# stablecabal/gyre

Hardware: AMD Instinct MI355X
Metric: SD1.5 512px 50-step images/sec (node) (higher is better)
Workload: dtype bf16

## Files before the change

gyre_amd/_lib.py:

```python
from __future__ import annotations

import ctypes as C
import os
from typing import Optional

import torch

_HERE = os.path.dirname(os.path.abspath(__file__))
MAX_LEVELS = 8

F32, BF16, F16 = 0, 1, 2
_TORCH_DTYPE = {torch.float32: F32, torch.bfloat16: BF16, torch.float16: F16}
LIB_PATHS = {BF16: os.environ.get("GYRE_HIP_LIB") or os.path.join(_HERE, "libgyre_hip.so"),
             F16: os.environ.get("GYRE_HIP_LIB_F16") or os.path.join(_HERE, "libgyre_hip_f16.so")}
LIB_PATH = LIB_PATHS[BF16]
_default_storage = F16 if os.environ.get("GYRE_STORAGE", "").lower() in ("f16", "fp16", "float16", "half") else BF16
STORAGE_TORCH_DTYPE = {BF16: torch.bfloat16, F16: torch.float16}


def default_storage() -> int:
    return _default_storage


def set_default_storage(storage: int) -> int:
# ... 139 lines not shown
    "gyre_op_repack_conv_weight": (_i, [_vp, _vp, _i, _i, _i, _i, _i, _vp]),
    "gyre_op_repack_conv_weight_scaled": (_i, [_vp, _vp, _i, _i, _i, _i, _i, _i, _f, _vp]),
    "gyre_op_repack_linear_weight": (_i, [_vp, _vp, _i, _i, _i, _vp]),
    "gyre_op_repack_bias": (_i, [_vp, _vp, _i, _i, _vp]),
    "gyre_op_repack_lora": (_i, [_vp, _vp, _i, _i, _i, _i, _i, _i, _i, _f, _i, C.POINTER(LoraPair), _vp]),
    "gyre_op_attention": (_i, [_vp, _vp, _i, _vp, _i, _vp, _i, _i, _i, _i, _i, _i, _vp, _i]),
    "gyre_op_qkv": (_i, [_vp, _vp, _i, _i, _vp, _i, _vp, _vp, _i]),
    "gyre_op_attention_ex": (_i, [_vp, _vp, _i, _vp, _i, _vp, _i, _i, _i, _i, _i, _i, _vp, _i, _i]),
    "gyre_op_groupnorm_bwd_workspace": (_sz, [_i, _i, _i, _i]),
    "gyre_op_groupnorm_bwd": (_i, [_vp, _vp, _vp, _i, _i, _i, _i, _i, _vp, _vp, _f, _i, _vp, _vp, _vp, _sz, _vp, _vp]),
    "gyre_op_layernorm_bwd": (_i, [_vp, _vp, _vp, _i, _i, _vp, _f, _vp, _vp]),
    "gyre_op_geglu_bwd": (_i, [_vp, _vp, _vp, _i, _i, _vp]),
    "gyre_op_attention_bwd_workspace": (_sz, [_i, _i, _i, _i, _i]),
    "gyre_op_attention_bwd": (_i, [_vp, _vp, _i, _vp, _i, _vp, _i, _vp, _i, _vp, _i, _i, _i, _i, _i, _i, _i, _vp, _sz,
                                   _vp, _i, _vp, _i, _vp, _i]),
    "gyre_op_tome_workspace": (_sz, [_i, _i, _i]),
    "gyre_op_tome_merge": (_i, [_vp, _vp, _i, _vp, _i, _i, _i, _i, _i, _vp, _sz, _vp, _vp, _i, _vp, _vp]),
    "gyre_op_tome_merge_ex": (_i, [_vp, _vp, _i, _vp, _i, _i, _i, _i, _i, _vp, _sz, _vp, _vp, _i, _vp, _vp, _vp, _vp]),
    "gyre_op_tome_unmerge": (_i, [_vp, _vp, _i, _i, _i, _i, _vp, _vp, _vp, _vp, _i]),
    "gyre_op_timestep_embedding": (_i, [_vp, _vp, _i, _i, _i, _f, _vp]),
    "gyre_op_rowvec_linear": (_i, [_vp, _vp, _i, _i, _vp, _vp, _i, _i, _vp, _i]),
    "gyre_op_timestep_linear": (_i, [_vp, _vp, _i, _i, _i, _f, _vp, _vp, _vp, _i, _vp, _i]),
    "gyre_op_cross_attention_block": (_i, [_vp, _vp, _i, _i, _i, _i, _vp, _vp, _f, _vp, _vp, _vp, _i, _i, _vp, _vp, _vp, _sz, _vp, _vp]),
    "gyre_op_nchw_to_nhwc": (_i, [_vp, _vp, _i, _i, _i, _i, _i, _vp]),
    "gyre_op_copy_probe": (_i, [_vp, _vp, _vp, _sz]),
    "gyre_op_pixel_unshuffle8": (_i, [_vp, _vp, _i, _i, _i, _i, _i, _vp]),
    "gyre_op_avgpool2": (_i, [_vp, _vp, _i, _i, _i, _i, _vp]),
    "gyre_op_relu": (_i, [_vp, _vp, _sz]),
}
EXPORTED_SYMBOLS = tuple(_SIGS)

_libs: dict = {}
import threading as _threading
_tls = _threading.local()


def lib(storage: Optional[int] = None) -> C.CDLL:
    storage = _default_storage if storage is None else storage
    l = _libs.get(storage)
    if l is None:
        path = LIB_PATHS[storage]
        if not os.path.exists(path):
            raise GyreError(f"{path} is missing: run `python -c 'import __graft_entry__ as g; g.build()'` "
                            f"(hipcc --offload-arch=gfx950).  There is no non-HIP fallback.")
        try:
            l = C.CDLL(path, mode=getattr(os, "RTLD_LOCAL", 0) | getattr(os, "RTLD_NOW", 2))
# ... 69 lines not shown
```

gyre_amd/build.py:

```python
from __future__ import annotations

import os
import subprocess
import sys
from concurrent.futures import ThreadPoolExecutor

HERE = os.path.dirname(os.path.abspath(__file__))
CSRC = os.path.join(HERE, "csrc")
LIB = os.path.join(HERE, "libgyre_hip.so")
LIB_F16 = os.path.join(HERE, "libgyre_hip_f16.so")
SOURCES = ["kernels_elem.hip", "kernels_gemm.hip", "kernels_gemm4s.hip", "kernels_gemm_ar.hip", "kernels_gemm_sm.hip", "kernels_conv_out.hip", "kernels_attn.hip", "kernels_xattn.hip", "kernels_tome.hip", "kernels_bwd.hip", "kernels_t2i.hip", "kernels_lora.hip", "model.hip", "model_vjp.hip", "model_t2i.hip"]
HEADERS = ["common.h", "kernels.h", "gemm_shared.h", "model_impl.h", os.path.join("..", "..", "include", "gyre_hip.h")]
FLAGS = ["--offload-arch=gfx950", "-O3", "-std=c++17", "-fPIC", "-mcode-object-version=5",
         "-Wno-unused-result", "-fno-gpu-rdc",
         "-mllvm", "-pragma-unroll-threshold=1000000"]


PER_FILE_FLAGS = {"kernels_attn.hip": ["-mllvm", "-amdgpu-mfma-vgpr-form=1"]}

RESOURCE_FILES = ("kernels_attn.hip", "kernels_gemm.hip", "kernels_gemm4s.hip", "kernels_gemm_ar.hip", "kernels_gemm_sm.hip")
SCRATCH_ALLOWED = ("k_attn3ILi80E", "k_gemm4s")
RESOURCES_JSON = os.path.join(HERE, "build", "kernel_resources.json")


def _hipcc() -> str:
    for c in (os.environ.get("HIPCC"), "/opt/rocm/bin/hipcc", "hipcc"):
        if c and (os.path.isabs(c) and os.path.exists(c) or not os.path.isabs(c)):
            return c
    raise RuntimeError("hipcc not found")


def _stale(out: str, deps) -> bool:
    if not os.path.exists(out):
        return True
    t = os.path.getmtime(out)
    return any(os.path.getmtime(d) > t for d in deps)


def _record_resources(source: str, remarks: str) -> None:
    import json
    import re
    import threading
    kernels, cur = {}, None
# ... 87 lines not shown
```

gyre_amd/csrc/kernels.h:

```cpp
#pragma once
#include "common.h"

int launch_nchw_to_nhwc(hipStream_t st, const void* x, int dtype, int B, int C, int HW, int Cpad, bf16_t* y);
int launch_add_nchw_into_nhwc(hipStream_t st, const void* r, int dtype, int B, int C, int HW, int Cpad, bf16_t* y);
int launch_ctx_to_bf16(hipStream_t st, const void* x, int dtype, size_t n, bf16_t* y);
int launch_dup_batch(hipStream_t st, const void* src, void* dst, size_t outer, size_t inner_bytes);
int launch_add_f32(hipStream_t st, float* y, const float* x, size_t n);
int launch_verify_hints(hipStream_t st, const int64_t* t, int B, int check_t, const void* x, size_t bytes_per_half, int check_pairs, int* flag);
int launch_timestep_embedding(hipStream_t st, const int64_t* t, int B, int dim, int flip, float shift, float* out);
int launch_rowvec_linear(hipStream_t st, float* x, int B, int K, const bf16_t* W, const float* bias, int N,
                         int act_in_silu, float* out, int ldo);
int launch_timestep_linear(hipStream_t st, const int64_t* t, int B, int dim, int flip, float shift, float* emb_scratch,
                           const bf16_t* W, const float* bias, int N, float* out, int ldo);

struct GnParams {
    const bf16_t* x; const bf16_t* x2; int C1;
    int B, HW, C, G;
    const float* gamma; const float* beta; float eps; int silu;
    float* partial;
    float* scale_shift;
    int nchunks;
    bf16_t* y;
    float* mean_rstd = nullptr;
    const float* cs_x = nullptr; int cs_x_chunks = 0;
// ... 7 lines not shown
long gemm_planner_state();
enum : int {
    GEMM_DBG_NO_SM            = 0x20,
    GEMM_DBG_SM_NO_SPLITK     = 0x40,
    GEMM_DBG_NO_SC_FOLD       = 0x80,
    GEMM_DBG_CONV_ZERO_PAGE   = 0x200,
    GEMM_DBG_NO_4S            = 0x400,
    GEMM_DBG_NO_LN_FOLD       = 0x800,
    GEMM_DBG_NO_GN_FOLD       = 0x1000,
    GEMM_DBG_NO_XATTN         = 0x2000,
    GEMM_DBG_NO_GEGLU_4S      = 0x4000,
    GEMM_DBG_LN_STATS_PASS    = 0x8000,
    GEMM_DBG_GEGLU_NO_LN_FOLD = 0x10000,
    GEMM_DBG_GN_STATS_PASS    = 0x20000,
    GEMM_DBG_NO_128x160       = 0x40000,
    GEMM_DBG_NO_CS_128x160    = 0x100000,
    GEMM_DBG_NO_AR            = 0x200000,
    GEMM_DBG_AR_ALL           = 0x400000,
    GEMM_DBG_NO_4S_128_TILES  = 0x800000,
    GEMM_DBG_TWO_STAGE_LINEAR = 0x1000000,
    GEMM_DBG_DEEP_RING        = 0x2000000,
    GEMM_DBG_NO_W_BLOCK       = 0x4000000,
    GEMM_DBG_TWO_STAGE_CONV   = 0x8000000,
};
int launch_groupnorm_stats(hipStream_t st, const GnParams& p);
int launch_groupnorm_apply(hipStream_t st, const GnParams& p);
bool gn_use_small(int HW, int C, int C1, int G);
bool gn_accepts_colstats(const GnParams& p);
int launch_groupnorm_small(hipStream_t st, const GnParams& p);
int launch_gn_fold(hipStream_t st, const GnParams& p, const bf16_t* W, const float* bias, int N, bf16_t* Wf, float* bf);
int launch_layernorm(hipStream_t st, const bf16_t* x, int M, int C, const float* gamma, const float* beta, float eps,
                     bf16_t* y);
int launch_layernorm_stats(hipStream_t st, const bf16_t* x, int M, int C, float eps, float* stats);

int launch_nhwc_to_nchw_f32(hipStream_t st, const bf16_t* x, int B, int C, int HW, int Cpad, float* y);
int launch_repack_conv(hipStream_t st, const void* w, int dtype, int O, int I, int KH, int KW, int Ipad, bf16_t* out,
                       float scale = 1.f);
int launch_repack_linear(hipStream_t st, const void* w, int dtype, int O, int I, int geglu_interleave, bf16_t* out);
int launch_cast_f32(hipStream_t st, const void* w, int dtype, size_t n, int geglu_interleave, float* out, float scale = 1.f);
int launch_copy_probe(hipStream_t st, const void* src, void* dst, size_t bytes);
#define GYRE_LORA_MAX_PAIRS 8
struct LoraArgs {
    const void* up[GYRE_LORA_MAX_PAIRS];
    const void* down[GYRE_LORA_MAX_PAIRS];
    int dtype[GYRE_LORA_MAX_PAIRS];
    int rank[GYRE_LORA_MAX_PAIRS];
// ... 102 lines not shown
    bool always_check = false;
    int ablation = 0;
    double flops = 0, bytes = 0;
};
AttnPlan attn_plan(const AttnParams& p, int variant);
constexpr int ATTN_PLAN_INTS = 12, ATTN_BWD_PLAN_INTS = 10;
int launch_attention(hipStream_t st, const AttnParams& p);

struct XattnParams {
    const bf16_t* x; int ldx;
    const bf16_t* wq;
    const float* q_colsum; const float* q_bias;
    const float* ln_parts; int ln_nparts; const float* ln_stats; float ln_eps;
    const bf16_t* k; const bf16_t* vt; int ldvt;
    const bf16_t* wo; const float* bo;
    bf16_t* out; int ldo;
    float* rowstat_out;
    int M, rows_per_sample, Nk, heads;
};

bool xattn_supports(int C, int heads, int Nq, int Nk, int M);
int launch_xattn(hipStream_t st, const XattnParams& p, int C);

struct GnBwdParams {
    const bf16_t* x; const bf16_t* x2; int C1;
    int B, HW, C, G;
    const float* gamma; const float* beta; float eps; int silu;
    const bf16_t* dy;
    const bf16_t* addend;
    bf16_t* dx; bf16_t* dx2;
    float* partial = nullptr; const float* fwd_partial = nullptr; int nchunks = 0;
};
size_t gn_bwd_workspace_bytes(int B, int HW, int C, int G);
int launch_groupnorm_bwd(hipStream_t st, GnBwdParams p, void* ws);
int launch_layernorm_bwd(hipStream_t st, const bf16_t* x, const bf16_t* dy, int M, int C, const float* gamma, float eps,
                         const bf16_t* addend, bf16_t* dx);
int launch_geglu_bwd(hipStream_t st, const bf16_t* pre, const bf16_t* dy, size_t M, int F, bf16_t* dpre);
int launch_pool2_sum(hipStream_t st, const bf16_t* du, int B, int H, int W, int Hu, int Wu, int C, bf16_t* dx);
int launch_zero_stuff2(hipStream_t st, const bf16_t* dy, int B, int Ho, int Wo, int H, int W, int C, bf16_t* dz);
int launch_add_bf16(hipStream_t st, bf16_t* y, const bf16_t* x, size_t n);
int launch_conv_weight_t(hipStream_t st, const bf16_t* w, int O, int I, bf16_t* wt);
int launch_transpose(hipStream_t st, const bf16_t* in, int ld_in, int R, int C, bf16_t* out, int ld_out, int batch,
                     size_t bs_in, size_t bs_out);
struct AttnBwdParams {
    const bf16_t* q; int ldq;
    const bf16_t* k; int ldk;
// ... 35 lines not shown
```

gyre_amd/csrc/model.hip:

```cpp
#include "model_impl.h"

static thread_local std::string g_err;
static thread_local int64_t g_launches = 0;
void gyre_set_error(const std::string& msg) { g_err = msg; }
int64_t& gyre_launch_counter() { return g_launches; }
extern "C" const char* gyre_last_error(void) { return g_err.c_str(); }
extern "C" int gyre_abi_version(void) { return GYRE_ABI_VERSION; }
extern "C" int gyre_storage_dtype(void) { return GYRE_STORAGE_DTYPE; }
extern "C" int64_t gyre_last_launch_count(void) { return g_launches; }

namespace {
struct ProfRec { hipEvent_t a, b; int kclass; double flops, bytes; };
struct ProfState {
    unsigned long long mask = 0;
    std::vector<ProfRec> recs;
    std::vector<std::pair<hipEvent_t, hipEvent_t>> pool;
};
thread_local ProfState g_prof;
static_assert(KC_COUNT <= 64, "profiler mask is 64 bits wide");
}
GyreProfScope::GyreProfScope(int kclass, hipStream_t st, double flops, double bytes) : st_(st) {
    if (!(g_prof.mask >> kclass & 1ull)) return;
    hipEvent_t a, b;
    if (!g_prof.pool.empty()) { a = g_prof.pool.back().first; b = g_prof.pool.back().second; g_prof.pool.pop_back(); }
// ... 752 lines not shown
                      int n_parts, void* ws, size_t ws_bytes, void* y) {
    if (!x || !w || !y || !gamma || !beta || !ws) GYRE_FAIL(GYRE_ERR_INVALID, "null argument");
    GemmParams p;
    if (qkv_tokens > 0 && (!vt_out || M % qkv_tokens || N != 3 * K || geglu)) GYRE_FAIL(GYRE_ERR_INVALID, "bad fused Q|K|V arguments");
    ln_linear_problem(p, M, K, N, geglu, qkv_tokens, ldt);
    p.A = (const bf16_t*)x; p.W = (const bf16_t*)w; p.bias = bias; p.out = y;
    if (qkv_tokens > 0) p.vt_out = (bf16_t*)vt_out;
    if (ws_bytes < gyre_op_ln_linear_workspace(p.N, K, M)) GYRE_FAIL(GYRE_ERR_WORKSPACE, "ln_linear: workspace too small");
    if (!gemm_plan(p).ln_fold) GYRE_FAIL(GYRE_ERR_UNSUPPORTED, "ln_linear: the planner's kernel for this shape cannot fold the LayerNorm");
    bf16_t* wf = (bf16_t*)ws;
    float* cs = (float*)((char*)ws + align_up((size_t)p.N * K * 2, 256));
    float* bb = (float*)((char*)cs + align_up((size_t)p.N * 4, 256));
    TRY(launch_ln_fold((hipStream_t)st, p.W, p.N, K, gamma, beta, bias, wf, cs, bb));
    if (row_parts && n_parts > 0) {
        p.ln_parts = row_parts; p.ln_nparts = n_parts; p.ln_eps = eps;
    } else {
        float* stats = (float*)((char*)bb + align_up((size_t)p.N * 4, 256));
        TRY(launch_layernorm_stats((hipStream_t)st, p.A, M, K, eps, stats));
        p.ln_stats = stats;
    }
    p.W = wf; p.bias = bb; p.ln_colsum = cs;
    return launch_gemm((hipStream_t)st, p);
}
int gyre_op_attention_ex(void* st, const void* q, int ldq, const void* k, int ldk, const void* vt, int ldvt, int B,
                         int heads, int Nq, int Nk, int D, void* o, int ldo, int k_prescaled) {
    if (!q || !k || !vt || !o) GYRE_FAIL(GYRE_ERR_INVALID, "null argument");
    AttnParams a;
    a.q = (const bf16_t*)q; a.ldq = ldq; a.k = (const bf16_t*)k; a.ldk = ldk; a.vt = (const bf16_t*)vt; a.ldvt = ldvt;
    a.o = (bf16_t*)o; a.ldo = ldo; a.B = B; a.H = heads; a.Nq = Nq; a.Nk = Nk; a.D = D; a.k_prescaled = k_prescaled ? 1 : 0;
    return launch_attention((hipStream_t)st, a);
}
int gyre_op_cross_attention_block(void* st, const void* x, int M, int tokens, int C, int heads, const float* gamma, const float* beta,
                                  float eps, const void* wq, const void* k, const void* vt, int Nk, int ldvt, const void* wo,
                                  const float* bo, void* ws, size_t ws_bytes, void* out, float* row_stats) {
    if (!x || !gamma || !beta || !wq || !k || !vt || !wo || !ws || !out) GYRE_FAIL(GYRE_ERR_INVALID, "null argument");
    if (tokens <= 0 || M % tokens) GYRE_FAIL(GYRE_ERR_INVALID, "cross_attention_block: M must be a multiple of tokens");
    if (!xattn_supports(C, heads, tokens, Nk, M)) GYRE_FAIL(GYRE_ERR_UNSUPPORTED, "cross_attention_block: shape outside the fused kernel's domain");
    if (ws_bytes < gyre_op_ln_linear_workspace(C, C, M)) GYRE_FAIL(GYRE_ERR_WORKSPACE, "cross_attention_block: workspace too small");
    bf16_t* wf = (bf16_t*)ws;
    float* cs = (float*)((char*)ws + align_up((size_t)C * C * 2, 256));
    float* bb = (float*)((char*)cs + align_up((size_t)C * 4, 256));
    float* stats = (float*)((char*)bb + align_up((size_t)C * 4, 256));
    TRY(launch_ln_fold((hipStream_t)st, (const bf16_t*)wq, C, C, gamma, beta, nullptr, wf, cs, bb));
    TRY(launch_layernorm_stats((hipStream_t)st, (const bf16_t*)x, M, C, eps, stats));
    XattnParams xp;
    xp.x = (const bf16_t*)x; xp.ldx = C; xp.wq = wf; xp.q_colsum = cs; xp.q_bias = bb;
// ... 16 lines not shown
```

gyre_amd/csrc/model_impl.h:

```cpp
#pragma once
#include "../../include/gyre_hip.h"
#include "kernels.h"
#include <cstdlib>
#include <cstdio>
#include <cmath>

#include <algorithm>
#include <array>
#include <cstring>
#include <map>
#include <memory>
#include <string>
#include <unordered_map>
#include <vector>

#define TRY(expr) do { int rc_ = (expr); if (rc_) return rc_; } while (0)
static inline size_t align_up(size_t v, size_t a) { return (v + a - 1) / a * a; }
static inline int pad8(int c) { return (c + 7) / 8 * 8; }

struct Arena {
    char* base = nullptr;
    size_t cap = 0, peak = 0;
    bool dry = false;
    std::map<size_t, size_t> free_;
// ... 559 lines not shown
        Store::LnEntry* e = store->ln_lookup(p.W, p.N, p.K, &fresh);
        if (!e) GYRE_FAIL(GYRE_ERR_HIP, "cannot allocate the LayerNorm-folded weight copy");
        if (!fresh) TRY(launch_ln_fold(st, p.W, p.N, p.K, ln.g, ln.b, p.bias, e->wf, e->cs, e->bb));
        p.W = e->wf; p.bias = e->bb; p.ln_colsum = e->cs;
        return 0;
    }
    int ln_linear(const Tn& x, const LnFold& ln, const bf16_t* w, int N, const float* bias, int geglu, bf16_t* y, int ldc) {
        GemmParams p;
        p.A = x.p; p.lda = x.C; p.mode = GEMM_LINEAR; p.W = w; p.K = x.C; p.N = N; p.M = x.rows(); p.bias = bias; p.geglu = geglu;
        p.out = y; p.ldc = ldc; p.out_mode = OUT_BF16; p.samples = batch; p.ar_ok = store != nullptr;
        if (store && gemm_plan(p).ln_fold) {
            Tn stats;
            TRY(ln_fold_into(p, ln, stats));
            int rc = run_gemm(p);
            free(stats);
            return rc;
        }
        Tn n;
        TRY(layernorm(x, ln.g, ln.b, n));
        p.A = n.p;
        int rc = run_gemm(p);
        free(n);
        return rc;
    }
    int mha(const Tn& xq_in, bool cross, const bf16_t* kvsrc, int kv_rows_per_batch, int kv_dim, const AttnW& w,
            const Tn& residual, Tn& out, MhaSave* sv = nullptr, const LnFold* ln = nullptr, RowStatBuf* rs_out = nullptr) {
        const int B = xq_in.B, Nq = xq_in.H * xq_in.W, C = w.c, D = C / w.heads;
        Tn q, k, vt, ao, nrm;
        Tn xq = xq_in;
        auto normalise = [&]() -> int {
            if (!ln) return 0;
            TRY(layernorm(xq_in, ln->g, ln->b, nrm));
            xq = nrm; ln = nullptr;
            return 0;
        };
        const bf16_t *qp, *kp, *vtp = nullptr; int ldq, ldk, Nk, ldvt;
        Tn km, vrow, tws;
        const int tr = (!cross && tome_r > 0 && Nq % 16 == 0) ? tome_effective_r(Nq, tome_r) : 0;
        if (!cross && tr > 0) {
            TRY(normalise());
            Nk = Nq - tr; ldvt = (Nk + 7) / 8 * 8;
            TRY(alloc(q, B, xq.H, xq.W, 2 * C));
            TRY(linear(xq.p, C, nullptr, 0, 0, B * Nq, C, w.wqk, 2 * C, w.bqk, nullptr, 0, 0, q.p, 2 * C));
            TRY(alloc(vrow, B, xq.H, xq.W, C));
            TRY(linear(xq.p, C, nullptr, 0, 0, B * Nq, C, w.wv, C, w.bv, nullptr, 0, 0, vrow.p, C));
            TRY(alloc(km, B, Nk, 1, C));
// ... 170 lines not shown
            if (!bs) {
                RowStatBuf rs1, rs2, rs3;
                const LnFold l1{bw.ln1g, bw.ln1b, &rs_h};
                TRY(mha(h, false, nullptr, 0, 0, bw.a1, h, h2, nullptr, &l1, &rs1));
                free(rs_h.t); rs_h.nparts = 0; free(h); h = h2;
                if (x_full && bi == 0) {
                    Tn hd;
                    TRY(dup_batch(h, hd));
                    free(h); h = hd;
                    if (rs1.nparts > 0) {
                        Tn rd;
                        TRY(alloc_raw(rd, 2 * rs1.t.bytes));
                        if (!dry()) TRY(launch_dup_batch(st, rs1.t.p, rd.p, rs1.nparts, (size_t)M * 2 * sizeof(float)));
                        free(rs1.t); rs1.t = rd;
                    }
                    TRY(dup_batch(x, *x_full));
                    x = *x_full;
                    batch = 2 * B; B = x.B; M = x.rows();
                }
                const LnFold l2{bw.ln2g, bw.ln2b, &rs1};
                TRY(mha(h, true, ctx.p, S, ctx_dim, bw.a2, h, h2, nullptr, &l2, &rs2));
                free(rs1.t); free(h); h = h2;
                const LnFold l3{bw.ln3g, bw.ln3b, &rs2};
                TRY(alloc(ff, B, x.H, x.W, 4 * C));
                TRY(ln_linear(h, l3, bw.ff1, 8 * C, bw.ff1b, 1, ff.p, 4 * C));
                free(rs2.t);
                TRY(alloc(h2, B, x.H, x.W, C));
                const bool more = bi + 1 < w.blocks.size();
                TRY(linear(ff.p, 4 * C, nullptr, 0, 0, M, 4 * C, bw.ff2, C, bw.ff2b, h.p, C, 0, h2.p, C, more ? &rs3 : nullptr));
                if (more) rs_h = rs3;
                free(ff); free(h);
                h = h2;
                continue;
            }
            TRY(layernorm(h, bw.ln1g, bw.ln1b, n));
            TRY(mha(n, false, nullptr, 0, 0, bw.a1, h, h2, bs ? &bs->a1 : nullptr));
            if (bs) { bs->h0 = h; bs->n1 = n; } else { free(n); free(h); }
            h = h2;
            TRY(layernorm(h, bw.ln2g, bw.ln2b, n));
            TRY(mha(n, true, ctx.p, S, ctx_dim, bw.a2, h, h2, bs ? &bs->a2 : nullptr));
            if (bs) { bs->h1 = h; bs->n2 = n; } else { free(n); free(h); }
            h = h2;
            TRY(layernorm(h, bw.ln3g, bw.ln3b, n));
            TRY(alloc(ff, B, x.H, x.W, 4 * C));
            TRY(linear(n.p, C, nullptr, 0, 0, M, C, bw.ff1, 8 * C, bw.ff1b, nullptr, 0, 1, ff.p, 4 * C));
            if (bs) bs->n3 = n; else free(n);
            TRY(alloc(h2, B, x.H, x.W, C));
            TRY(linear(ff.p, 4 * C, nullptr, 0, 0, M, 4 * C, bw.ff2, C, bw.ff2b, h.p, C, 0, h2.p, C));
            free(ff);
            if (bs) bs->h2 = h; else free(h);
            h = h2;
// ... 594 lines not shown
```

include/gyre_hip.h:

```cpp
#ifndef GYRE_HIP_H
#define GYRE_HIP_H

#include <stddef.h>
#include <stdint.h>

#ifdef __cplusplus
extern "C" {
#endif

#define GYRE_ABI_VERSION 1

typedef enum { GYRE_F32 = 0, GYRE_BF16 = 1, GYRE_F16 = 2 } gyre_dtype;

typedef enum {
    GYRE_OK = 0,
    GYRE_ERR_INVALID = -1,
    GYRE_ERR_KEY = -2,
    GYRE_ERR_INCOMPLETE = -3,
    GYRE_ERR_WORKSPACE = -4,
    GYRE_ERR_HIP = -5,
    GYRE_ERR_UNSUPPORTED = -6
} gyre_status;

#define GYRE_MAX_LEVELS 8
// ... 122 lines not shown
int gyre_t2i_set_weight(gyre_t2i* h, const char* key, const void* dev_ptr, int dtype, const int64_t* shape, int ndim, void* stream);
int gyre_t2i_finalize(gyre_t2i* h, void* stream);
size_t gyre_t2i_workspace_bytes(gyre_t2i* h, int B, int H, int W);
int gyre_t2i_forward(gyre_t2i* h, void* stream, const void* image_nchw, int in_dtype, int B, int H, int W,
                     void* workspace, size_t workspace_bytes, void* const* features_out_nchw, int n, int out_dtype);

int gyre_prof_set_mask(unsigned long long mask);
int gyre_prof_num_classes(void);
const char* gyre_prof_class_name(int kclass);
int gyre_prof_collect(int64_t* launches, double* ms, double* flops, double* bytes);

int gyre_debug_force_gemm_cfg(int cfg);
int gyre_debug_set_splitk_workspace(void* ws_dev, size_t bytes);
int gyre_debug_set_ar_workspace(void* ws_dev, size_t bytes);
int gyre_debug_set_wblk_workspace(void* ws_dev, size_t bytes);
int gyre_debug_force_attn_variant(int v);
long gyre_debug_attn_redo_count(void);
int gyre_debug_attn_plan(int B, int H, int Nq, int Nk, int D, int k_prescaled, int ldq, int ldk, int ldvt, int ldo, int32_t* out);
int gyre_debug_attn_bwd_plan(int B, int H, int Nq, int Nk, int D, int with_dk, int32_t* out);
int gyre_debug_attn_tables(int which, int32_t* out, int cap);
int gyre_debug_xattn_stamps(void* dev_buf);
int gyre_debug_gemm_ablation(int bits);
int gyre_debug_ln_linear_folds(int M, int K, int N, int geglu);
int gyre_debug_gn_uses_small(int HW, int C, int C1, int groups);
typedef struct gyre_gemm_test_args {
    int32_t conv, M, K, N, geglu;
    int32_t B, Hi, Wi, Cin, stride, pad, ups, Hup, Wup, wrap;
    int32_t C1, lda, lda2, ldc, ldr;
    int32_t rows_per_sample, ld_rowbias, samples;
    int32_t out_mode, out_dtype, tokens, ldt;
    int32_t colstat_unit;
    const void* A; const void* A2; const void* W;
    const float* bias; const float* rowbias; const void* residual;
    void* out; void* ws; size_t ws_bytes;
    const void* sc_A; const void* sc_A2; int32_t sc_K, sc_C1, sc_lda, sc_lda2;
} gyre_gemm_test_args;
int gyre_op_gemm_test(void* stream, const gyre_gemm_test_args* a);
int gyre_debug_gemm_plan(const gyre_gemm_test_args* a, int32_t* out);
int gyre_debug_gemm_tiles(int32_t* out, int cap);

int gyre_set_batch_invariant(int canonical_samples);
int gyre_get_batch_invariant(void);

int gyre_op_groupnorm(void* stream, const void* x, const void* x2, int C1, int B, int HW, int C, int groups,
                      const float* gamma, const float* beta, float eps, int silu,
                      void* workspace, size_t workspace_bytes, void* y);
size_t gyre_op_groupnorm_workspace(int B, int HW, int C, int groups);
size_t gyre_op_gemm_splitk_bytes(int conv, int M, int N, int K, int B);
int gyre_op_conv3x3_colstats(void* stream, const void* x, int B, int Hi, int Wi, int Cin, const void* w_repacked, int Cout,
                             const float* bias, const void* residual, int stride, int ups, int unit, void* y, float* stats_out,
                             size_t stats_bytes, void* workspace, size_t workspace_bytes, int* rows_out);
int gyre_op_linear_colstats(void* stream, const void* x, int M, int K, const void* w_bf16_rowmajor, int N, const float* bias,
                            const void* residual, int rows_per_sample, int unit, void* y, float* stats_out, size_t stats_bytes,
                            void* workspace, size_t workspace_bytes, int* rows_out);
int gyre_op_groupnorm_colstats(void* stream, const void* x, const void* x2, int C1, int B, int HW, int C, int groups,
                               const float* gamma, const float* beta, float eps, int silu, const float* cs_x, int cs_x_chunks,
                               const float* cs_x2, int cs_x2_chunks, int unit, void* workspace, size_t workspace_bytes, void* y);
int gyre_op_gn_fold(void* stream, const void* x, int B, int HW, int C, int groups, const float* gamma, const float* beta, float eps,
                    const void* W, const float* bias, int N, const float* cs_x, int cs_x_chunks, int unit,
                    void* workspace, size_t workspace_bytes, void* Wf_out, float* bf_out);
int gyre_op_layernorm(void* stream, const void* x, int M, int C, const float* gamma, const float* beta,
                      float eps, void* y);
int gyre_op_linear(void* stream, const void* x, int M, int K, const void* w_bf16_rowmajor, int N,
                   const float* bias, const void* residual, int geglu, void* y);
size_t gyre_op_ln_linear_workspace(int w_rows, int K, int M);
int gyre_op_ln_linear(void* stream, const void* x, int M, int K, const float* gamma, const float* beta, float eps,
                      const void* w_bf16_rowmajor, int N, const float* bias, int geglu, int qkv_tokens, void* vt_out, int ldt,
                      const float* row_parts, int n_parts, void* workspace, size_t workspace_bytes, void* y);
int gyre_op_linear_rowstats_parts(int M, int K, int N, int has_residual);
int gyre_op_linear_rowstats(void* stream, const void* x, int M, int K, const void* w_bf16_rowmajor, int N, const float* bias,
                            const void* residual, void* y, float* stats_out);
int gyre_op_linear_t(void* stream, const void* x, int M, int K, const void* w_bf16_rowmajor, int N,
                     const float* bias, int tokens_per_batch, int ldt, void* y);
int gyre_op_conv3x3(void* stream, const void* x, int B, int Hi, int Wi, int Cin, const void* w_krsc, int Cout,
                    const float* bias, const void* residual, int stride, int ups, int asym, void* y);
int gyre_op_conv3x3_shortcut(void* stream, const void* x, int B, int H, int W, int Cin, const void* w_krsc, int Cout, const float* bias,
                             const void* sx, int C1, const void* sx2, int C2, const void* w_sc, const float* bias_sc, void* ws,
                             size_t ws_bytes, void* y);
int gyre_op_conv3x3_nchw(void* stream, const void* x, int B, int H, int W, int Cin, const void* w_krsc, int Cout,
                         const float* bias, void* y, int y_dtype, int force_tiles);
int gyre_op_repack_conv_weight(void* stream, const float* w_oihw, int Cout, int Cin, int KH, int KW, int Cin_pad,
                               void* w_krsc_bf16);
int gyre_op_repack_conv_weight_scaled(void* stream, const void* w_oihw, int dtype, int Cout, int Cin, int KH, int KW, int Cin_pad,
                                      float scale, void* w_krsc);
int gyre_op_repack_linear_weight(void* stream, const float* w_oi, int O, int I, int geglu_interleave, void* w_bf16);
int gyre_op_repack_bias(void* stream, const float* b, int n, int geglu_interleave, float* out);
int gyre_op_repack_lora(void* stream, const void* base, int base_dtype, int O, int I, int KH, int KW, int I_pad,
                        int geglu_interleave, float scale_p, int n_pairs, const gyre_lora_pair* pairs, void* out);
int gyre_op_attention(void* stream, const void* q, int ldq, const void* k, int ldk, const void* vt, int ldvt,
                      int B, int heads, int Nq, int Nk, int D, void* o, int ldo);
int gyre_op_qkv(void* stream, const void* x, int M, int C, const void* w_qkv, int tokens, void* qk_out, void* vt_out, int ldt);
// ... 47 lines not shown
```

Measured before the change: 9.096.

## Fuse feed-forward GEGLU and down-projection into one streaming kernel for C=320

Adds a fused kernel that computes the LN-folded FF1 GEMM, the GEGLU activation with a polynomial erf, and the FF2 GEMM in one pass. The 1280-wide hidden activation stays in registers and is never written to HBM. Weights are pre-packed into stages and streamed through double-buffered LDS with direct global-to-LDS loads. The goal is to remove the hidden-tensor write and read and one kernel launch per transformer block at 320 channels. The path only triggers when there are no row stats for a next block (the last block of each stack), M/128 is at least 256, and LN folding applies, so coverage is narrow.

```diff
diff --git a/gyre_amd/_lib.py b/gyre_amd/_lib.py
--- a/gyre_amd/_lib.py
+++ b/gyre_amd/_lib.py
@@ -185,6 +185,9 @@
     "gyre_op_rowvec_linear": (_i, [_vp, _vp, _i, _i, _vp, _vp, _i, _i, _vp, _i]),
     "gyre_op_timestep_linear": (_i, [_vp, _vp, _i, _i, _i, _f, _vp, _vp, _vp, _i, _vp, _i]),
     "gyre_op_cross_attention_block": (_i, [_vp, _vp, _i, _i, _i, _i, _vp, _vp, _f, _vp, _vp, _vp, _i, _i, _vp, _vp, _vp, _sz, _vp, _vp]),
+    "gyre_op_ff_pair_workspace": (_sz, [_i]),
+    "gyre_op_ff_pair": (_i, [_vp, _vp, _i, _i, _vp, _vp, _f, _vp, _i, _vp, _vp, _vp, _vp, _vp, _vp, _sz, _vp, C.POINTER(C.c_int)]),
+    "gyre_debug_ff_pair_plan": (_i, [_i, _i, _i, _i, _i, C.POINTER(C.c_int32)]),
     "gyre_op_nchw_to_nhwc": (_i, [_vp, _vp, _i, _i, _i, _i, _i, _vp]),
     "gyre_op_copy_probe": (_i, [_vp, _vp, _vp, _sz]),
     "gyre_op_pixel_unshuffle8": (_i, [_vp, _vp, _i, _i, _i, _i, _i, _vp]),
diff --git a/gyre_amd/build.py b/gyre_amd/build.py
--- a/gyre_amd/build.py
+++ b/gyre_amd/build.py
@@ -9,7 +9,7 @@
 CSRC = os.path.join(HERE, "csrc")
 LIB = os.path.join(HERE, "libgyre_hip.so")
 LIB_F16 = os.path.join(HERE, "libgyre_hip_f16.so")
-SOURCES = ["kernels_elem.hip", "kernels_gemm.hip", "kernels_gemm4s.hip", "kernels_gemm_ar.hip", "kernels_gemm_sm.hip", "kernels_conv_out.hip", "kernels_attn.hip", "kernels_xattn.hip", "kernels_tome.hip", "kernels_bwd.hip", "kernels_t2i.hip", "kernels_lora.hip", "model.hip", "model_vjp.hip", "model_t2i.hip"]
+SOURCES = ["kernels_elem.hip", "kernels_gemm.hip", "kernels_gemm4s.hip", "kernels_gemm_ar.hip", "kernels_ffpair.hip", "kernels_gemm_sm.hip", "kernels_conv_out.hip", "kernels_attn.hip", "kernels_xattn.hip", "kernels_tome.hip", "kernels_bwd.hip", "kernels_t2i.hip", "kernels_lora.hip", "model.hip", "model_vjp.hip", "model_t2i.hip"]
 HEADERS = ["common.h", "kernels.h", "gemm_shared.h", "model_impl.h", os.path.join("..", "..", "include", "gyre_hip.h")]
 FLAGS = ["--offload-arch=gfx950", "-O3", "-std=c++17", "-fPIC", "-mcode-object-version=5",
          "-Wno-unused-result", "-fno-gpu-rdc",
@@ -18,7 +18,7 @@
 
 PER_FILE_FLAGS = {"kernels_attn.hip": ["-mllvm", "-amdgpu-mfma-vgpr-form=1"]}
 
-RESOURCE_FILES = ("kernels_attn.hip", "kernels_gemm.hip", "kernels_gemm4s.hip", "kernels_gemm_ar.hip", "kernels_gemm_sm.hip")
+RESOURCE_FILES = ("kernels_attn.hip", "kernels_gemm.hip", "kernels_gemm4s.hip", "kernels_gemm_ar.hip", "kernels_ffpair.hip", "kernels_gemm_sm.hip")
 SCRATCH_ALLOWED = ("k_attn3ILi80E", "k_gemm4s")
 RESOURCES_JSON = os.path.join(HERE, "build", "kernel_resources.json")
 
diff --git a/gyre_amd/csrc/kernels.h b/gyre_amd/csrc/kernels.h
--- a/gyre_amd/csrc/kernels.h
+++ b/gyre_amd/csrc/kernels.h
@@ -53,6 +53,7 @@
     GEMM_DBG_DEEP_RING        = 0x2000000,
     GEMM_DBG_NO_W_BLOCK       = 0x4000000,
     GEMM_DBG_TWO_STAGE_CONV   = 0x8000000,
+    GEMM_DBG_NO_FFPAIR        = 0x10000000,
 };
 int launch_groupnorm_stats(hipStream_t st, const GnParams& p);
 int launch_groupnorm_apply(hipStream_t st, const GnParams& p);
@@ -201,6 +202,24 @@
 bool xattn_supports(int C, int heads, int Nq, int Nk, int M);
 int launch_xattn(hipStream_t st, const XattnParams& p, int C);
 
+struct FfPairParams {
+    const bf16_t* x = nullptr; int ldx = 0;
+    const void* w_packed = nullptr;
+    const float* colsum1 = nullptr; const float* bias1 = nullptr;
+    const float* ln_parts = nullptr; int ln_nparts = 0; const float* ln_stats = nullptr; float ln_eps = 1e-5f;
+    const float* bias2 = nullptr;
+    const bf16_t* residual = nullptr; int ldr = 0;
+    bf16_t* out = nullptr; int ldo = 0;
+    int M = 0, C = 320;
+};
+bool ffpair_supports(int C, int hidden, int M, int rows_per_sample);
+bool ffpair_plan(int C, int hidden, int M, int rows_per_sample, bool want_rowstats, bool ln_folded);
+size_t ffpair_packed_bytes();
+int ffpair_lds_bytes();
+void ffpair_ff1_problem(GemmParams& p, int C, int M, int samples);
+int launch_ffpair_pack(hipStream_t st, const bf16_t* W1, const bf16_t* W2, void* out);
+int launch_ffpair(hipStream_t st, const FfPairParams& p);
+
 struct GnBwdParams {
     const bf16_t* x; const bf16_t* x2; int C1;
     int B, HW, C, G;
diff --git a/gyre_amd/csrc/kernels_ffpair.hip b/gyre_amd/csrc/kernels_ffpair.hip
--- /dev/null
+++ b/gyre_amd/csrc/kernels_ffpair.hip
@@ -0,0 +1,285 @@
+#include "gemm_shared.h"
+#include <atomic>
+#include <type_traits>
+
+namespace {
+typedef __attribute__((address_space(3))) char fp_lds_char_t;
+typedef __attribute__((ext_vector_type(4))) unsigned fp_u32x4;
+template <int V> using fp_ic = std::integral_constant<int, V>;
+template <int I, int N, typename F>
+__device__ __forceinline__ void fp_static_for(F&& f) {
+    if constexpr (I < N) { f(fp_ic<I>{}); fp_static_for<I + 1, N>(f); }
+}
+__device__ __forceinline__ void fp_glds(unsigned lds_addr, const void* vptr) {
+    asm volatile("s_mov_b32 m0, %0\n\ts_nop 0\n\tglobal_load_lds_dwordx4 %1, off" ::"s"(lds_addr), "v"(vptr) : "memory");
+}
+constexpr int FP_C = 320, FP_HID = 1280;
+constexpr int FP_NCH = FP_HID / 32;
+constexpr int FP_NST = FP_NCH + 1;
+constexpr int FP_W1B = 64 * FP_C * 2, FP_W2B = FP_C * 32 * 2, FP_STAGE = FP_W1B + FP_W2B;
+constexpr int FP_NF1 = FP_W1B / 1024, FP_NF2 = FP_W2B / 1024, FP_NF = FP_NF1 + FP_NF2;
+constexpr int FP_ROWS = 2 * FP_HID;
+constexpr int FP_PATCH = 160 + 4;
+constexpr int FP_LDS = 2 * FP_STAGE + 2 * FP_ROWS * 4;
+static_assert(8 * 16 * FP_PATCH * 4 <= 2 * FP_STAGE && FP_LDS <= 160 * 1024, "LDS budget");
+
+__host__ __device__ __forceinline__ int fp_w1_row(int c, int tile, int r) {
+    const int hl = 8 * (r >> 2) + (r & 3) + 4 * (tile & 1);
+    return 64 * c + 32 * (hl >> 4) + (hl & 15) + 16 * (tile >> 1);
+}
+}
+
+__global__ __launch_bounds__(256) void k_ffpair_pack(const bf16_t* W1, const bf16_t* W2, uint4* out) {
+    constexpr int per = FP_STAGE / 16;
+    const int idx = blockIdx.x * 256 + threadIdx.x;
+    if (idx >= FP_NST * per) return;
+    const int s = idx / per, r = idx - s * per;
+    uint4 v = make_uint4(0u, 0u, 0u, 0u);
+    if (r < FP_NF1 * 64) {
+        const int f = r >> 6, l = r & 63, ks = f >> 2, tile = f & 3;
+        if (s < FP_NCH) v = *(const uint4*)(W1 + (size_t)fp_w1_row(s, tile, l & 15) * FP_C + 32 * ks + 8 * (l >> 4));
+    } else {
+        const int r2 = r - FP_NF1 * 64, nt = r2 >> 6, l = r2 & 63;
+        if (s >= 1) v = *(const uint4*)(W2 + (size_t)(16 * nt + (l & 15)) * FP_HID + 32 * (s - 1) + 8 * (l >> 4));
+    }
+    out[idx] = v;
+}
+
+template <int RG>
+__global__ __launch_bounds__(512 / RG, RG == 1 ? 2 : 1) void k_gemm_ar_pair(FfPairParams p) {
+    constexpr int NW = 8 / RG, NT = NW * 64;
+    extern __shared__ __attribute__((aligned(16))) char smem[];
+    const int tid = threadIdx.x, lane = tid & 63;
+    const int w = __builtin_amdgcn_readfirstlane(tid >> 6);
+    const int fr = lane & 15, fq = lane >> 4;
+    const int mw = blockIdx.x * 128 + w * 16 * RG;
+    const unsigned lds0 = (unsigned)(size_t)(fp_lds_char_t*)smem;
+    float* cb = (float*)(smem + 2 * FP_STAGE);
+    float* cc = cb + FP_ROWS;
+
+    const char* wsrc = (const char*)p.w_packed + lane * 16;
+    auto issue = [&](int s, int slot) {
+        const char* src = wsrc + (size_t)s * FP_STAGE;
+        const unsigned d = lds0 + slot * FP_STAGE;
+#pragma unroll
+        for (int i = 0; i < FP_NF / NW; ++i) fp_glds(d + (w + NW * i) * 1024, src + (w + NW * i) * 1024);
+        if constexpr (FP_NF % NW != 0) {
+            if (w < FP_NF % NW) fp_glds(d + (w + FP_NF / NW * NW) * 1024, src + (w + FP_NF / NW * NW) * 1024);
+        }
+    };
+    issue(0, 0);
+
+    bf16x8_t xf[RG][10];
+#pragma unroll
+    for (int rg = 0; rg < RG; ++rg) {
+        const bf16_t* xrow = p.x + (size_t)(mw + rg * 16 + fr) * p.ldx + 8 * fq;
+#pragma unroll
+        for (int ks = 0; ks < 10; ++ks) xf[rg][ks] = __builtin_bit_cast(bf16x8_t, *(const uint4*)(xrow + 32 * ks));
+    }
+    for (int i = tid; i < FP_ROWS; i += NT) {
+        const int src = fp_w1_row(i >> 6, (i >> 4) & 3, i & 15);
+        cb[i] = p.bias1[src];
+        cc[i] = p.colsum1[src];
+    }
+    float lrstd[RG], lrmu[RG];
+#pragma unroll
+    for (int rg = 0; rg < RG; ++rg) {
+        const int m = mw + rg * 16 + fr;
+        if (p.ln_nparts > 0) {
+            float su = 0.f, sq = 0.f;
+            for (int t = 0; t < p.ln_nparts; ++t) {
+                const float2 v = ((const float2*)p.ln_parts)[(size_t)t * p.M + m];
+                su += v.x; sq += v.y;
+            }
+            const float invk = 1.0f / (float)p.C;
+            const float mean = su * invk;
+            lrstd[rg] = 1.0f / sqrtf(fmaxf(sq * invk - mean * mean, 0.f) + p.ln_eps);
+            lrmu[rg] = lrstd[rg] * mean;
+        } else {
+            const float2 rs = ((const float2*)p.ln_stats)[m];
+            lrstd[rg] = rs.x; lrmu[rg] = rs.y;
+        }
+    }
+
+    f32x4_t accX[RG][4], accY[RG][4];
+    f32x4_t out[RG][20];
+    const f32x4_t zero4 = {0.f, 0.f, 0.f, 0.f};
+#pragma unroll
+    for (int rg = 0; rg < RG; ++rg)
+#pragma unroll
+        for (int nt = 0; nt < 20; ++nt) out[rg][nt] = zero4;
+
+    float4 kvb, kvc, kgb, kgc;
+    float eo[8];
+    float ev = 0.f, eg = 0.f, ez = 0.f, ep = 0.f;
+    fp_u32x4 hf[RG];
+#pragma unroll
+    for (int rg = 0; rg < RG; ++rg) hf[rg] = fp_u32x4{0u, 0u, 0u, 0u};
+    constexpr int NSTG = 19;
+    auto epi_stage = [&](auto s_c, auto rg_c, int c, const f32x4_t (&a)[4]) {
+        constexpr int S = decltype(s_c)::value, rg = decltype(rg_c)::value;
+        auto f4 = [](const float4& v, int i) { return i == 0 ? v.x : i == 1 ? v.y : i == 2 ? v.z : v.w; };
+        if constexpr (S == 0 || S == 9) {
+            constexpr int t = S == 0 ? 0 : 1;
+            const float4* b4 = (const float4*)cb + c * 16 + fq;
+            const float4* c4 = (const float4*)cc + c * 16 + fq;
+            kvb = b4[t * 4]; kgb = b4[(t + 2) * 4];
+            kvc = c4[t * 4]; kgc = c4[(t + 2) * 4];
+        } else if constexpr (S < 18) {
+            constexpr int q = S < 9 ? S - 1 : S - 10, t = S < 9 ? 0 : 1, i = q >> 1, e = 4 * t + i;
+            if constexpr ((q & 1) == 0) {
+                ev = fmaf(a[t][i], lrstd[rg], fmaf(-lrmu[rg], f4(kvc, i), f4(kvb, i)));
+                eg = fmaf(a[t + 2][i], lrstd[rg], fmaf(-lrmu[rg], f4(kgc, i), f4(kgb, i)));
+                ez = fabsf(eg) * 0.70710678118654752f;
+                ep = fmaf(ez, 0.0000430638f, 0.0002765672f);
+                ep = fmaf(ez, ep, 0.0001520143f);
+                ep = fmaf(ez, ep, 0.0092705272f);
+            } else {
+                ep = fmaf(ez, ep, 0.0422820123f);
+                ep = fmaf(ez, ep, 0.0705230784f);
+                ep = fmaf(ez, ep, 1.0f);
+                ep *= ep; ep *= ep; ep *= ep; ep *= ep;
+                const float rq = __builtin_amdgcn_rcpf(ep);
+                eo[e] = ev * fmaf(-0.70710678118654752f * ez, rq, fmaxf(eg, 0.f));
+            }
+        } else {
+            hf[rg] = fp_u32x4{pack_bf16x2(eo[0], eo[1]), pack_bf16x2(eo[2], eo[3]), pack_bf16x2(eo[4], eo[5]), pack_bf16x2(eo[6], eo[7])};
+        }
+    };
+
+    constexpr int PF = 6, RING = 8;
+    auto body = [&](int s, int slot, f32x4_t (&cur)[RG][4], const f32x4_t (&prev)[RG][4], auto mode_tag) {
+        constexpr int MODE = decltype(mode_tag)::value;
+        constexpr int I0 = MODE == 2 ? FP_NF1 : 0, I1 = MODE == 0 ? FP_NF1 : FP_NF;
+        const char* sb = smem + slot * FP_STAGE + lane * 16;
+        bf16x8_t wf[RING];
+        fp_static_for<I0, I0 + PF>([&](auto i_c) {
+            constexpr int i = decltype(i_c)::value;
+            wf[i % RING] = *(const bf16x8_t*)(sb + i * 1024);
+        });
+        if constexpr (MODE == 2) {
+            fp_static_for<0, RG>([&](auto rg_c) {
+                fp_static_for<0, NSTG>([&](auto s_c) { epi_stage(s_c, rg_c, s - 1, prev[decltype(rg_c)::value]); });
+            });
+            __builtin_amdgcn_sched_barrier(0);
+        }
+        fp_static_for<I0, I1>([&](auto i_c) {
+            constexpr int i = decltype(i_c)::value;
+            if constexpr (i + PF < I1) wf[(i + PF) % RING] = *(const bf16x8_t*)(sb + (i + PF) * 1024);
+            fp_static_for<0, RG>([&](auto rg_c) {
+                constexpr int rg = decltype(rg_c)::value;
+                if constexpr (i < FP_NF1) {
+                    constexpr int ks = i >> 2, tile = i & 3;
+                    cur[rg][tile] = GYRE_MFMA_16x16x32(wf[i % RING], xf[rg][ks], ks == 0 ? zero4 : cur[rg][tile], 0, 0, 0);
+                    constexpr int j = i * RG + rg, S2 = j / 2;
+                    if constexpr (MODE == 1 && (j & 1) == 0 && S2 < NSTG * RG)
+                        epi_stage(fp_ic<S2 % NSTG>{}, fp_ic<S2 / NSTG>{}, s - 1, prev[S2 / NSTG]);
+                } else {
+                    constexpr int nt = i - FP_NF1;
+                    out[rg][nt] = GYRE_MFMA_16x16x32(wf[i % RING], __builtin_bit_cast(bf16x8_t, hf[rg]), out[rg][nt], 0, 0, 0);
+                }
+                __builtin_amdgcn_sched_barrier(0);
+            });
+        });
+    };
+    auto top = [&](int s, int slot) {
+        asm volatile("s_waitcnt vmcnt(0) lgkmcnt(0)" ::: "memory");
+        __builtin_amdgcn_s_barrier();
+        __builtin_amdgcn_sched_barrier(0);
+        if (s + 1 < FP_NST) issue(s + 1, slot ^ 1);
+    };
+    using mode0 = fp_ic<0>; using mode1 = fp_ic<1>; using mode2 = fp_ic<2>;
+
+    __syncthreads();
+    top(0, 0);
+    body(0, 0, accX, accY, mode0{});
+    for (int s = 1; s + 1 < FP_NCH; s += 2) {
+        top(s, 1);
+        body(s, 1, accY, accX, mode1{});
+        top(s + 1, 0);
+        body(s + 1, 0, accX, accY, mode1{});
+    }
+    top(FP_NCH - 1, 1);
+    body(FP_NCH - 1, 1, accY, accX, mode1{});
+    top(FP_NCH, 0);
+    uint4 rres[RG][2][5];
+    if (p.residual) {
+#pragma unroll
+        for (int rg = 0; rg < RG; ++rg)
+#pragma unroll
+            for (int h = 0; h < 2; ++h)
+#pragma unroll
+                for (int q = 0; q < 5; ++q) {
+                    const int v = lane + 64 * q, row = v / 20, c8 = v - row * 20;
+                    rres[rg][h][q] = *(const uint4*)(p.residual + (size_t)(mw + rg * 16 + row) * p.ldr + h * 160 + c8 * 8);
+                }
+    }
+    body(FP_NCH, 0, accX, accY, mode2{});
+
+    __syncthreads();
+    float* my = (float*)smem + w * (16 * FP_PATCH);
+#pragma unroll
+    for (int rg = 0; rg < RG; ++rg)
+#pragma unroll
+        for (int h = 0; h < 2; ++h) {
+#pragma unroll
+            for (int jj = 0; jj < 10; ++jj) {
+                const int nt = h * 10 + jj;
+                float4 o = make_float4(out[rg][nt][0], out[rg][nt][1], out[rg][nt][2], out[rg][nt][3]);
+                if (p.bias2) { const float4 bv = *(const float4*)(p.bias2 + nt * 16 + 4 * fq); o.x += bv.x; o.y += bv.y; o.z += bv.z; o.w += bv.w; }
+                *(float4*)(my + fr * FP_PATCH + jj * 16 + 4 * fq) = o;
+            }
+#pragma unroll
+            for (int q = 0; q < 5; ++q) {
+                const int v = lane + 64 * q, row = v / 20, c8 = v - row * 20;
+                const float4 lo = *(const float4*)(my + row * FP_PATCH + c8 * 8);
+                const float4 hi = *(const float4*)(my + row * FP_PATCH + c8 * 8 + 4);
+                float f[8] = {lo.x, lo.y, lo.z, lo.w, hi.x, hi.y, hi.z, hi.w};
+                if (p.residual) {
+                    float r[8];
+                    unpack8(rres[rg][h][q], r);
+#pragma unroll
+                    for (int e = 0; e < 8; ++e) f[e] += r[e];
+                }
+                *(uint4*)(p.out + (size_t)(mw + rg * 16 + row) * p.ldo + h * 160 + c8 * 8) = pack8(f);
+            }
+        }
+}
+
+bool ffpair_supports(int C, int hidden, int M, int rows_per_sample) {
+    return C == FP_C && hidden == FP_HID && M > 0 && M % 128 == 0 && rows_per_sample > 0 && rows_per_sample % 128 == 0;
+}
+bool ffpair_plan(int C, int hidden, int M, int rows_per_sample, bool want_rowstats, bool ln_folded) {
+    if (!ffpair_supports(C, hidden, M, rows_per_sample) || M / 128 < 256 || want_rowstats || !ln_folded) return false;
+    if (gemm_get_batch_invariant() > 0 || (gemm_planner_state() & GEMM_DBG_NO_FFPAIR)) return false;
+    return true;
+}
+size_t ffpair_packed_bytes() { return (size_t)FP_NST * FP_STAGE; }
+int ffpair_lds_bytes() { return FP_LDS; }
+void ffpair_ff1_problem(GemmParams& p, int C, int M, int samples) {
+    p.A = (const bf16_t*)(uintptr_t)256; p.lda = C; p.mode = GEMM_LINEAR; p.W = (const bf16_t*)(uintptr_t)256; p.K = C; p.N = 8 * C; p.M = M;
+    p.geglu = 1; p.out = (void*)(uintptr_t)256; p.ldc = 4 * C; p.out_mode = OUT_BF16; p.samples = samples; p.ar_ok = 1;
+}
+int launch_ffpair_pack(hipStream_t st, const bf16_t* W1, const bf16_t* W2, void* out) {
+    const int total = FP_NST * (FP_STAGE / 16);
+    hipLaunchKernelGGL(k_ffpair_pack, dim3((total + 255) / 256), dim3(256), 0, st, W1, W2, (uint4*)out);
+    GYRE_LAUNCH_CHECK();
+    return 0;
+}
+int launch_ffpair(hipStream_t st, const FfPairParams& p) {
+    if (p.M <= 0 || p.M % 128 || p.C != FP_C) GYRE_FAIL(-6, "ff_pair: C = 320 and M a positive multiple of 128");
+    if (!p.x || !p.w_packed || !p.colsum1 || !p.bias1 || !p.out || (!p.ln_stats && p.ln_nparts <= 0))
+        GYRE_FAIL(-1, "ff_pair: null argument");
+    if ((p.ldx % 8) || (p.ldo % 8) || (p.residual && p.ldr % 8) || p.ldx < FP_C || p.ldo < FP_C || (p.residual && p.ldr < FP_C) ||
+        ((((size_t)p.x | (size_t)p.out | (size_t)p.residual | (size_t)p.w_packed | (size_t)p.bias2) & 15) != 0))
+        GYRE_FAIL(-1, "ff_pair: operands must be 16-byte aligned with strides that are multiples of 8 elements");
+    const double fl = 2.0 * p.M * ((double)FP_ROWS * FP_C + (double)FP_C * FP_HID);
+    const double by = (double)p.M * FP_C * 2.0 * (p.residual ? 3.0 : 2.0) + ((double)FP_ROWS * FP_C + (double)FP_C * FP_HID) * 2.0;
+    GyreProfScope prof_(KC_GEMM_AR, st, fl, by);
+    static std::atomic<unsigned long long> attr_done{0};
+    if (gyre_lds_attr_needed(attr_done))
+        (void)hipFuncSetAttribute((const void*)k_gemm_ar_pair<1>, hipFuncAttributeMaxDynamicSharedMemorySize, FP_LDS);
+    hipLaunchKernelGGL(k_gemm_ar_pair<1>, dim3(p.M / 128), dim3(512), FP_LDS, st, p);
+    GYRE_LAUNCH_CHECK();
+    return 0;
+}
diff --git a/gyre_amd/csrc/model.hip b/gyre_amd/csrc/model.hip
--- a/gyre_amd/csrc/model.hip
+++ b/gyre_amd/csrc/model.hip
@@ -798,6 +798,61 @@
     p.W = wf; p.bias = bb; p.ln_colsum = cs;
     return launch_gemm((hipStream_t)st, p);
 }
+size_t gyre_op_ff_pair_workspace(int M) {
+    if (M <= 0) return 0;
+    return gyre_op_ln_linear_workspace(2560, 320, M) + align_up(ffpair_packed_bytes(), 256) + align_up((size_t)M * 1280 * 2, 256);
+}
+int gyre_op_ff_pair(void* st_, const void* x, int M, int rows_per_sample, const float* gamma, const float* beta, float eps,
+                    const float* row_parts, int n_parts, const void* w1, const float* b1, const void* w2, const float* b2,
+                    const void* residual, void* ws, size_t ws_bytes, void* y, int* fused_out) {
+    if (!x || !gamma || !beta || !w1 || !b1 || !w2 || !ws || !y) GYRE_FAIL(GYRE_ERR_INVALID, "null argument");
+    if (M <= 0 || rows_per_sample <= 0 || M % rows_per_sample) GYRE_FAIL(GYRE_ERR_INVALID, "ff_pair: M must be a positive multiple of rows_per_sample");
+    if (ws_bytes < gyre_op_ff_pair_workspace(M)) GYRE_FAIL(GYRE_ERR_WORKSPACE, "ff_pair: workspace too small");
+    hipStream_t st = (hipStream_t)st_;
+    const int C = 320, R = 2560;
+    bf16_t* wf = (bf16_t*)ws;
+    float* cs = (float*)((char*)ws + align_up((size_t)R * C * 2, 256));
+    float* bb = (float*)((char*)cs + align_up((size_t)R * 4, 256));
+    float* stats = (float*)((char*)bb + align_up((size_t)R * 4, 256));
+    char* pk = (char*)ws + gyre_op_ln_linear_workspace(R, C, M);
+    bf16_t* hidden = (bf16_t*)(pk + align_up(ffpair_packed_bytes(), 256));
+    TRY(launch_ln_fold(st, (const bf16_t*)w1, R, C, gamma, beta, b1, wf, cs, bb));
+    const bool parts = row_parts && n_parts > 0;
+    if (!parts) TRY(launch_layernorm_stats(st, (const bf16_t*)x, M, C, eps, stats));
+    const bool fused = ffpair_supports(C, 4 * C, M, rows_per_sample) && !(gemm_planner_state() & GEMM_DBG_NO_FFPAIR);
+    if (fused_out) *fused_out = fused ? 1 : 0;
+    if (fused) {
+        TRY(launch_ffpair_pack(st, wf, (const bf16_t*)w2, pk));
+        FfPairParams f;
+        f.x = (const bf16_t*)x; f.ldx = C; f.w_packed = pk; f.colsum1 = cs; f.bias1 = bb;
+        if (parts) { f.ln_parts = row_parts; f.ln_nparts = n_parts; } else f.ln_stats = stats;
+        f.ln_eps = eps; f.bias2 = b2; f.residual = (const bf16_t*)residual; f.ldr = C; f.out = (bf16_t*)y; f.ldo = C; f.M = M; f.C = C;
+        return launch_ffpair(st, f);
+    }
+    GemmParams p;
+    ln_linear_problem(p, M, C, 4 * C, 1, 0, 0);
+    p.A = (const bf16_t*)x; p.W = wf; p.bias = bb; p.ln_colsum = cs; p.out = hidden;
+    if (parts) { p.ln_parts = row_parts; p.ln_nparts = n_parts; p.ln_eps = eps; } else p.ln_stats = stats;
+    GemmPlan pl = gemm_plan(p);
+    if (!pl.ln_fold) { pl = GemmPlan(); pl.cfg = 7; pl.ln_fold = true; }
+    TRY(launch_gemm(st, p, pl));
+    GemmParams q;
+    q.A = hidden; q.lda = 4 * C; q.mode = GEMM_LINEAR; q.W = (const bf16_t*)w2; q.K = 4 * C; q.N = C; q.M = M; q.bias = b2;
+    q.residual = (const bf16_t*)residual; q.ldr = C; q.out = y; q.ldc = C; q.out_mode = OUT_BF16;
+    return launch_gemm(st, q);
+}
+int gyre_debug_ff_pair_plan(int C, int hidden, int M, int rows_per_sample, int want_rowstats, int32_t* out) {
+    if (!out) GYRE_FAIL(GYRE_ERR_INVALID, "ff_pair_plan: null output");
+    if (C <= 0 || hidden <= 0 || M <= 0 || rows_per_sample <= 0 || M % rows_per_sample) GYRE_FAIL(GYRE_ERR_INVALID, "ff_pair_plan: bad sizes");
+    GemmParams p;
+    ffpair_ff1_problem(p, C, M, M / rows_per_sample);
+    const bool folds = gemm_plan(p).ln_fold;
+    out[0] = ffpair_plan(C, hidden, M, rows_per_sample, want_rowstats != 0, folds) ? 1 : 0;
+    out[1] = ffpair_supports(C, hidden, M, rows_per_sample) ? 1 : 0;
+    out[2] = folds ? 1 : 0;
+    out[3] = M / 128; out[4] = ffpair_lds_bytes(); out[5] = (int32_t)ffpair_packed_bytes();
+    return 0;
+}
 int gyre_op_attention_ex(void* st, const void* q, int ldq, const void* k, int ldk, const void* vt, int ldvt, int B,
                          int heads, int Nq, int Nk, int D, void* o, int ldo, int k_prescaled) {
     if (!q || !k || !vt || !o) GYRE_FAIL(GYRE_ERR_INVALID, "null argument");
diff --git a/gyre_amd/csrc/model_impl.h b/gyre_amd/csrc/model_impl.h
--- a/gyre_amd/csrc/model_impl.h
+++ b/gyre_amd/csrc/model_impl.h
@@ -605,6 +605,33 @@
         int rc = run_gemm(p);
         free(n);
         return rc;
+    }
+    int ff_pair(const Tn& x, const LnFold& ln, const bf16_t* w1, const float* b1, const bf16_t* w2, const float* b2, bool more, Tn& y,
+                bool* ran) {
+        *ran = false;
+        const int C = x.C, M = x.rows();
+        if (!store || tiling) return 0;
+        GemmParams p;
+        ffpair_ff1_problem(p, C, M, batch);
+        if (!ffpair_plan(C, 4 * C, M, x.H * x.W, more, gemm_plan(p).ln_fold)) return 0;
+        p.A = x.p; p.W = w1; p.bias = b1;
+        Tn stats;
+        TRY(ln_fold_into(p, ln, stats));
+        TRY(alloc(y, x.B, x.H, x.W, C));
+        if (!dry()) {
+            bool fresh = false;
+            void* pk = store->ar_lookup(w2, ffpair_packed_bytes(), &fresh, 33);
+            if (!pk) GYRE_FAIL(GYRE_ERR_HIP, "cannot allocate the packed weight copy of the fused feed-forward pair");
+            if (!fresh) TRY(launch_ffpair_pack(st, p.W, w2, pk));
+            FfPairParams f;
+            f.x = x.p; f.ldx = C; f.w_packed = pk; f.colsum1 = p.ln_colsum; f.bias1 = p.bias;
+            f.ln_parts = p.ln_parts; f.ln_nparts = p.ln_nparts; f.ln_stats = p.ln_stats; f.ln_eps = p.ln_eps;
+            f.bias2 = b2; f.residual = x.p; f.ldr = C; f.out = y.p; f.ldo = C; f.M = M; f.C = C;
+            TRY(launch_ffpair(st, f));
+        }
+        free(stats);
+        *ran = true;
+        return 0;
     }
     int mha(const Tn& xq_in, bool cross, const bf16_t* kvsrc, int kv_rows_per_batch, int kv_dim, const AttnW& w,
             const Tn& residual, Tn& out, MhaSave* sv = nullptr, const LnFold* ln = nullptr, RowStatBuf* rs_out = nullptr) {
@@ -821,11 +848,18 @@
                 TRY(mha(h, true, ctx.p, S, ctx_dim, bw.a2, h, h2, nullptr, &l2, &rs2));
                 free(rs1.t); free(h); h = h2;
                 const LnFold l3{bw.ln3g, bw.ln3b, &rs2};
+                const bool more = bi + 1 < w.blocks.size();
+                bool pair = false;
+                TRY(ff_pair(h, l3, bw.ff1, bw.ff1b, bw.ff2, bw.ff2b, more, h2, &pair));
+                if (pair) {
+                    free(rs2.t); free(h);
+                    h = h2;
+                    continue;
+                }
                 TRY(alloc(ff, B, x.H, x.W, 4 * C));
                 TRY(ln_linear(h, l3, bw.ff1, 8 * C, bw.ff1b, 1, ff.p, 4 * C));
                 free(rs2.t);
                 TRY(alloc(h2, B, x.H, x.W, C));
-                const bool more = bi + 1 < w.blocks.size();
                 TRY(linear(ff.p, 4 * C, nullptr, 0, 0, M, 4 * C, bw.ff2, C, bw.ff2b, h.p, C, 0, h2.p, C, more ? &rs3 : nullptr));
                 if (more) rs_h = rs3;
                 free(ff); free(h);
diff --git a/include/gyre_hip.h b/include/gyre_hip.h
--- a/include/gyre_hip.h
+++ b/include/gyre_hip.h
@@ -168,6 +168,7 @@
 int gyre_debug_xattn_stamps(void* dev_buf);
 int gyre_debug_gemm_ablation(int bits);
 int gyre_debug_ln_linear_folds(int M, int K, int N, int geglu);
+int gyre_debug_ff_pair_plan(int C, int hidden, int M, int rows_per_sample, int want_rowstats, int32_t* out);
 int gyre_debug_gn_uses_small(int HW, int C, int C1, int groups);
 typedef struct gyre_gemm_test_args {
     int32_t conv, M, K, N, geglu;
@@ -213,6 +214,10 @@
 int gyre_op_ln_linear(void* stream, const void* x, int M, int K, const float* gamma, const float* beta, float eps,
                       const void* w_bf16_rowmajor, int N, const float* bias, int geglu, int qkv_tokens, void* vt_out, int ldt,
                       const float* row_parts, int n_parts, void* workspace, size_t workspace_bytes, void* y);
+size_t gyre_op_ff_pair_workspace(int M);
+int gyre_op_ff_pair(void* stream, const void* x, int M, int rows_per_sample, const float* gamma, const float* beta, float eps,
+                    const float* row_parts, int n_parts, const void* w1_geglu_rowmajor, const float* b1_geglu, const void* w2_rowmajor,
+                    const float* b2, const void* residual, void* workspace, size_t workspace_bytes, void* y, int* fused_out);
 int gyre_op_linear_rowstats_parts(int M, int K, int N, int has_residual);
 int gyre_op_linear_rowstats(void* stream, const void* x, int M, int K, const void* w_bf16_rowmajor, int N, const float* bias,
                             const void* residual, void* y, float* stats_out);
```

After: 9.168 (median of 6 runs). About the same (+0.8%).
